# zz9tf/multimodal-fusion

Measured on AMD Instinct MI355X. Metric: similarity-pairs/sec (NxN cosine+top-k), higher is better.
Workload: dtype f16 MFMA scan + f32 exact re-rank; 1 GPU; N=262144 d=512 single-modality cosine + top-5, self excluded, f32 features, unit-norm Gaussian rows; rows_per_rank=262144, parallelism=single GPU, driver=single, scan_kernel=scan_b16x<f16> (v_mfma_f32_16x16x32_f16), col_splits=1, scan_grid=3088, fallback_rows=0, overflow_rows=0, query_order=False, near_duplicate_rows_estimate=0

## Files before the change

multimodal-fusion_amd/csrc/mmf_api.hip:

```cpp
#include <stdarg.h>
#include <string.h>

#include <algorithm>
#include <map>
#include <mutex>
#include <optional>
#include <utility>
#include <vector>

#include "mmf_host.h"

namespace mmf {

static thread_local char g_err[512] = "";

void set_error(const char* fmt, ...) {
  va_list ap;
  va_start(ap, fmt);
  vsnprintf(g_err, sizeof(g_err), fmt, ap);
  va_end(ap);
}

struct WsEntry { char* base = nullptr; size_t cap = 0; WsKept kept; };
static std::mutex g_ws_mu;
// ... 624 lines not shown
      else MMF_TRY(launch_scan_b16(sp, splits, L, scan_scratch, pn, s, &grid));
    } else {
      int list_base = 0;
      for (int p = 0; p < fo.n_panels; ++p) {
        const mmf_panel& P = fo.panels[p];
        if (P.ready_event) MMF_HIP(hipStreamWaitEvent(s, static_cast<hipEvent_t>(P.ready_event), 0));
        MMF_TRY(t_panel[p].start(profile, s));
        pn.list_base = list_base;
        list_base += 2 * panel_splits[p];
        pn.seg_len = (uint32_t)P.seg_len; pn.seg_stride = (uint32_t)P.seg_stride; pn.id_off = (uint32_t)P.id_base;
        sp.ZC = P.Z; sp.cb = P.cb; sp.m = P.m; sp.m_pad = P.m_pad;
        MMF_TRY(launch_scan_b16(sp, panel_splits[p], L, scan_scratch, pn, s, &grid));
        MMF_TRY(t_panel[p].stop(s));
      }
    }
    MMF_TRY(launch_scan_b16_audit(pn, L.overflow, n, s));
    if (const char* e = getenv("MMF_DEBUG_FLAG_ROWS")) {
      const int64_t f = atoll(e);
      if (f > 0) MMF_HIP(hipMemsetAsync(L.overflow, 1, (size_t)(f < n ? f : n) * 4, s));
    }
    MMF_TRY(t_scan.stop(s));
    if (symmetric && getenv("MMF_SYMMETRIC_DEBUG")) {
      MMF_HIP(hipStreamSynchronize(s));
      std::vector<uint32_t> hc((size_t)n), hl((size_t)sym_grid() * 8), hr((size_t)sym_grid() * 8);
      uint32_t none = 0;
      MMF_HIP(hipMemcpy(hc.data(), sym_cnt, hc.size() * 4, hipMemcpyDeviceToHost));
      MMF_HIP(hipMemcpy(hl.data(), sym.val_cnt, hl.size() * 4, hipMemcpyDeviceToHost));
      MMF_HIP(hipMemcpy(hr.data(), sym.log_cnt, hr.size() * 4, hipMemcpyDeviceToHost));
      MMF_HIP(hipMemcpy(&none, sym.none_cnt, 4, hipMemcpyDeviceToHost));
      unsigned long long tot = 0, logged = 0, records = 0; uint32_t mx = 0, lmx = 0;
      for (uint32_t v : hc) { tot += v; if (v > mx) mx = v; }
      for (uint32_t v : hl) logged += v;
      for (uint32_t v : hr) { records += v; if (v > lmx) lmx = v; }
      bool live, forward;
      symmetric_live_mode(&live, &forward);
      int phases; bool antipodal;
      symmetric_schedule_mode(&phases, &antipodal, sym_G);
      const size_t first_b = (size_t)sym_schedule_phase_b_begin((n + 255) / 256, sym_G) * 8;
      unsigned long long logged_b = 0;
      for (size_t i = first_b; i < hl.size(); ++i) logged_b += hl[i];
      fprintf(stderr, "[mmf symmetric] G %d grid %lld %s %s: rows without a threshold %u, received entries %llu (%.1f per row, largest %u of %d), fullest wave log %u of %d, logged entries %llu (%.1f per row, filing %s), records %llu, phases %d antipodal %d, logged by phase B %llu (%.1f per row)\n",
              sym_G, (long long)sym_grid(), live ? "live" : "frozen", forward ? "ahead" : "back", none, tot, (double)tot / (double)n, mx,
              kSymCap, lmx, scan_b16_sym_log_cap(), logged, (double)logged / (double)n, symmetric_prune_mode() ? "pruned" : "complete", records,
              forward ? 1 : phases, (antipodal && !forward) ? 1 : 0, logged_b, (double)logged_b / (double)n);
    }
    if (select_wait_event) MMF_HIP(hipStreamWaitEvent(s, static_cast<hipEvent_t>(select_wait_event), 0));

    SelectProblem q = r.select();
    q.rx = fo.rx; q.cy = fo.cy; q.perm = fo.perm;
    q.fail_rows = flags.fail_rows; q.fail_count = flags.fail_count; q.cand_total = r.stats ? flags.cand_total : nullptr;
    q.two_pass = true;
    q.order_scratch = getenv("MMF_SELECT_UNORDERED") ? nullptr : order_scratch;
    q.out_stride = out_stride;
    if (leave_floors) { q.floor_key_out = floor_key_out; q.floor_id_out = floor_id_out; }
    MMF_TRY(t_sel.start(profile, s));
    MMF_TRY(launch_select(q, L, s));
    MMF_TRY(t_sel.stop(s));

    MMF_TRY(flags.read(r.stats != nullptr, s));
    const uint32_t* h_fail4 = flags.h_fail4;
    const uint32_t h_fail = h_fail4[0];
    failed_rows = h_fail;
    if (h_fail > 0 && getenv("MMF_DEBUG_PRINT_FLAGGED")) {
      const uint32_t nshow = h_fail < 8 ? h_fail : 8;
      int32_t rows[8];
      MMF_HIP(hipMemcpy(rows, flags.fail_rows, nshow * sizeof(int32_t), hipMemcpyDeviceToHost));
      for (uint32_t i = 0; i < nshow; ++i) {
// ... 3898 lines not shown
```

multimodal-fusion_amd/csrc/mmf_host.h:

```cpp
#pragma once
#include <hip/hip_runtime.h>
#include <functional>
#include <optional>
#include <stdint.h>
#include <stdio.h>

#include <string>
#include <vector>

#include "../../include/mmf_hg.h"
#include "../../include/mmf_hg_topk.h"
#include "../../include/mmf_hg_topk16.h"
#include "../../include/ext/mmf_hg_topk16_seg.h"
#include "../../include/ext/mmf_hg_topk_xy.h"
#include "../../include/ext/mmf_hg_seg_exact.h"
#include "../../include/ext/mmf_hg_topk_anyk.h"
#include "../../include/ext/mmf_hg_kmeans_ragged.h"
#include "../../include/ext/mmf_hg_cross_seg.h"
#include "../../include/ext/mmf_hg_cross_seg16.h"
#include "../../include/ext/mmf_hg_cross_segw.h"
#include "../../include/ext/mmf_hg_fast_anyk.h"
#include "../../include/ext/mmf_hg_wide_anyk.h"
#include "../../include/ext/mmf_hg_seg_anyk.h"
#include "../../include/ext/mmf_hg_cross_seg_anyk.h"
// ... 129 lines not shown
  int spill_cap = 0;
  int spill_stacks = 0;
  uint32_t* sym_cnt = nullptr;
  uint2* sym_ent = nullptr;
  int sym_cap = 0;
};

constexpr int kSymListPairs = 3;
int64_t sym_schedule_grid(int64_t nb, int G);
int64_t sym_schedule_phase_b_begin(int64_t nb, int G);
void sym_schedule_table(int64_t nb, int G, int launch, int32_t* out, bool forward = false, int phases = 1, bool antipodal = false);
int sym_default_group(int64_t nb);
constexpr int kSymCap = 512;
constexpr int kSymLogPerWave = 2304;
int scan_b16_sym_log_cap();
struct SymBuffers {
  float* thr = nullptr;
  uint32_t* log = nullptr;
  uint32_t* log_cnt = nullptr;
  uint32_t* val_cnt = nullptr;
  int32_t* sched = nullptr;
  uint32_t* none_cnt = nullptr;
  static size_t bytes(int64_t n_pad, int64_t grid) {
    return ws_bytes(n_pad, 4) + ws_bytes((size_t)grid * 8 * kSymLogPerWave * 16, 4) + 2 * ws_bytes((size_t)grid * 8, 4) +
           ws_bytes((size_t)grid * 16, 4) + ws_bytes(4, 4);
  }
  void carve(Workspace& ws, int64_t n_pad, int64_t grid) {
    thr = ws.take<float>(n_pad); log = ws.take<uint32_t>((size_t)grid * 8 * kSymLogPerWave * 16);
    log_cnt = ws.take<uint32_t>((size_t)grid * 8); val_cnt = ws.take<uint32_t>((size_t)grid * 8); sched = ws.take<int32_t>((size_t)grid * 16); none_cnt = ws.take<uint32_t>(4);
  }
};

struct ScanB16Panel {
  int list_base = 0;
  uint32_t seg_len = 0, seg_stride = 0, id_off = 0;
  int32_t* seed = nullptr;
  int64_t seed_stride = 0;
  int share = 0;
  int32_t* sunk = nullptr;
};

int64_t prep_f32_rows(int64_t n);
int64_t prep_f32_dim(int64_t d);
size_t prep_f32_bytes(int64_t n, int64_t d);
int launch_prep_f32(const void* X, int64_t n, int64_t d, int dtype, const int32_t* row_ids, float* out, hipStream_t s);

struct ScanProblem {
  const void* X; int64_t n;
  const void* Y; int64_t m;
  const float* Xp = nullptr;
  const float* Yp = nullptr;
  int64_t d;
// ... 307 lines not shown
```

multimodal-fusion_amd/csrc/mmf_scan_bf16.hip:

```cpp
#include <stdlib.h>

#include <type_traits>

#include "mmf_dev.h"
#include "mmf_host.h"

namespace mmf {

constexpr int B_CT = 32;
#ifndef MMF_B_CAP
#define MMF_B_CAP 15
#endif
constexpr int B_CAP = MMF_B_CAP;
constexpr int B_CAP_BIG = 16;
constexpr int B_CAP_WIDE = 32;

typedef __bf16 bf16x8_t __attribute__((ext_vector_type(8)));
typedef _Float16 f16x8_t __attribute__((ext_vector_type(8)));
typedef uint32_t u32x4 __attribute__((ext_vector_type(4)));

struct PrepArgs {
  const void* X; int64_t n; int64_t d; int dtype; int metric;
  const float* scal;
  const uint32_t* max_n;
// ... 173 lines not shown
  const float g_chain = (float)(d + 2) * 5.9604645e-8f;
  const float slot_eps = (cap <= 16) ? 1.9073486e-6f : 3.8146973e-6f;
  const float e1 = rn * ZB + un * RB + (g_acc + slot_eps) * (zn * ZB + CB);
  float e2;
  if (metric == MMF_DOT) e2 = g_chain * un * UB;
  else if (metric == MMF_COSINE) e2 = (g_chain + 4.7683716e-7f) * un * UB * 1.01f;
  else e2 = g_chain * un * UB + 2.3841858e-7f * (un * un + UB * UB);
  return 2.0f * (e1 + e2) * 1.001f + 1e-30f;
}

__device__ __forceinline__ void glds4(const void* gptr, const void* lptr) {
  __builtin_amdgcn_global_load_lds((const __attribute__((address_space(1))) void*)(gptr), (__attribute__((address_space(3))) void*)(lptr), 4, 0, 0);
}

#ifndef MMF_SYM_ABLATE
#define MMF_SYM_ABLATE 0
#endif
#ifndef MMF_SYM_EARLY_THR
#define MMF_SYM_EARLY_THR 1
#endif
#ifndef MMF_SYM_RECORDS
#define MMF_SYM_RECORDS 1
#endif
#ifndef MMF_SYM_SCALAR_ANY
#define MMF_SYM_SCALAR_ANY 1
#endif
#ifndef MMF_SYM_ABLATE_Q
#define MMF_SYM_ABLATE_Q 0
#endif
#ifndef MMF_SYM_COUNT
#define MMF_SYM_COUNT 0
#endif
template <int KS, bool F16, bool DBG, int NW, int TPB, int CAP, bool SPLITK = false, bool SEG = false, int SYM = 0, bool XSEG = false,
          bool CEIL = false>
__global__ __launch_bounds__(64 * NW, (NW == 8) ? 2 : 1) void scan_b16x_kernel(ScanB16Args a) {
  static_assert(!CEIL || (SYM == 0 && !DBG), "per-row ceilings: the plain and the table-driven schedules (SEG, XSEG) only");
  static_assert(!SPLITK || (TPB == 1 && NW == 8 && (KS % 8) == 0), "split-k pairs");
  static_assert(SYM == 0 || (!SPLITK && !SEG && !DBG && TPB == 2), "symmetric schedule: the d = 512 kernel only");
  static_assert(!XSEG || (SEG && SYM == 0 && !DBG), "the cross-segment mask rides on the table-driven schedule");
  constexpr int NQW = SPLITK ? NW / 2 : NW;
  constexpr int NTL = 64 * NQW;
  constexpr int QT = 32 * NQW;
  constexpr int STAGES = 2 * TPB;
  constexpr int ROWB = KS * 32;
  constexpr int TILEB = B_CT * ROWB;
  constexpr int PIECES = TILEB / 1024;
// ... 70 lines not shown
    const float UB = __uint_as_float(a.maxima[2]), CB = __uint_as_float(a.maxima[3]);
    const float zn = a.q_zn[qop], rn = a.q_rn[qop], un = a.q_un[qop];
    const float g_acc = (float)(KS * 16 + 8) * 5.9604645e-8f;
    const float g_chain = (float)(a.d + 2) * 5.9604645e-8f;
    const float slot_eps = (CAP <= 16) ? 1.9073486e-6f : 3.8146973e-6f;
    const float e1 = rn * ZB + un * RB + (g_acc + slot_eps) * (zn * ZB + CB);
    float e2;
    if (a.metric == MMF_DOT) e2 = g_chain * un * UB;
    else if (a.metric == MMF_COSINE) e2 = (g_chain + 4.7683716e-7f) * un * UB * 1.01f;
    else e2 = g_chain * un * UB + 2.3841858e-7f * (un * un + UB * UB);
    margin = 2.0f * (e1 + e2) * 1.001f + 1e-30f;
  }

  SlotList<CAP, NTL> list;
  list.init(lkeys + (tid & (NTL - 1)), lids + (tid & (NTL - 1)));
  if (!qvalid) list.thr = __builtin_huge_valf();
  else if (a.spill_cnt) {
    list.sink.cnt = a.spill_cnt; list.sink.ids = a.spill_ids; list.sink.cap = (uint32_t)a.spill_cap; list.sink.row = qpos;
    list.sink.seg_len = a.seg_len; list.sink.seg_stride = a.seg_stride; list.sink.id_off = id_off;
    if (DBG) list.sink.ablate = (a.debug & 128) ? 1 : 0;
    if (a.spill_stacks) list.sink.stacks = 1 + half;
  }
  float pub = -kFltMax;
  auto sync_seed = [&]() {
    if (!qvalid) return;
    bool rose = false;
    if (list.thr > pub && list.thr > list.lost) {
      pub = list.thr;
      atomicMax(a.seed + qpos, seed_enc(pub));
      rose = true;
    }
    if (!a.share) return;
    const int32_t o = __hip_atomic_load(a.seed + qpos, __ATOMIC_RELAXED, __HIP_MEMORY_SCOPE_AGENT);
    if (o > kSeedNone) {
      const float t = __int_as_float(o >= 0 ? o : (o ^ 0x7fffffff));
      if (t > list.thr) { list.thr = t; pub = t; }
    }
    if constexpr (SYM == 2) {
      if (rose && a.sym_live) __hip_atomic_store(a.sym_thr + qpos, list.thr, __ATOMIC_RELAXED, __HIP_MEMORY_SCOPE_AGENT);
    }
  };
  constexpr bool SCALAR_ANY = SYM != 0 && MMF_SYM_SCALAR_ANY != 0;
  auto sym_hits = [&](unsigned long long b) -> bool { asm("" : "+s"(b)); return b != 0ull; };
  if (a.share) sync_seed();
  const bool seeded = !__any(list.thr == -kFltMax);

  constexpr int KS2 = SPLITK ? KS / 4 : KS / 2;
  const int kbyte = khalf * KS2 * 64;
  u32x4 qf[KS2][2];
  {
    const char* qbase = reinterpret_cast<const char*>(a.ZQ) + (q0 + 32 * qw + c16) * (int64_t)ROWB + g * 16 + kbyte;
#pragma unroll
    for (int s = 0; s < KS2; ++s) {
      qf[s][0] = *reinterpret_cast<const u32x4*>(qbase + s * 64);
      qf[s][1] = *reinterpret_cast<const u32x4*>(qbase + 16 * (int64_t)ROWB + s * 64);
    }
#pragma unroll
    for (int s = 0; s < KS2; ++s) { asm volatile("" : "+v"(qf[s][0])); asm volatile("" : "+v"(qf[s][1])); }
  }

  int lo[4];
#pragma unroll
  for (int j = 0; j < 4; ++j) lo[j] = c16 * ROWB + ((((4 * j + g) ^ c16) & 15) << 4);
// ... 6 lines not shown
    const int r = off / ROWB;
    const int chunk = (off % ROWB) >> 4;
    const int src_chunk = (chunk & ~15) | ((chunk ^ r) & 15);
    src_off[i] = (uint32_t)(r * ROWB + src_chunk * 16);
  }
  const char* zc0 = reinterpret_cast<const char*>(a.ZC) + (SYM != 0 ? 0 : t_begin * (int64_t)TILEB);
  const char* cb0 = reinterpret_cast<const char*>(a.cb + (SYM != 0 ? 0 : t_begin * B_CT));
  const char* zt0 = SYM != 0 ? zc0 + t_begin * (int64_t)TILEB : zc0;
  const char* ct0 = SYM != 0 ? cb0 + t_begin * B_CT * 4 : cb0;
  const __amdgpu_buffer_rsrc_t zrsrc = __builtin_amdgcn_make_buffer_rsrc(const_cast<char*>(zc0), 0, -1, 0x00020000);
  auto issue_piece = [&](const char* tsrc, int stage, int i) {
    if (DBG && (a.debug & 2)) return;
    if (DBG && (a.debug & 32)) tsrc = zc0;
    __builtin_amdgcn_raw_ptr_buffer_load_lds(zrsrc, (__attribute__((address_space(3))) void*)(tiles + stage * TILEB + (wave + NW * i) * 1024),
                                             16, (int)src_off[i], (int)(uint32_t)(tsrc - zc0), 0, 0);
  };
  const __amdgpu_buffer_rsrc_t brsrc = __builtin_amdgcn_make_buffer_rsrc(const_cast<char*>(cb0), 0, -1, 0x00020000);
  auto issue_bias = [&](const char* bsrc, int stage) {
    const uint32_t l = __builtin_amdgcn_mbcnt_hi(~0u, __builtin_amdgcn_mbcnt_lo(~0u, 0u));
    if (l < 32)
      __builtin_amdgcn_raw_ptr_buffer_load_lds(brsrc, (__attribute__((address_space(3))) void*)(cbs + stage * 64), 4, (int)(l * 4u),
                                               (int)(uint32_t)(bsrc - cb0), 0, 0);
  };
  auto sym_thr_stage = [&](int stage) -> float* { return lkeys + CAP * NTL + stage * 32; };
  auto issue_thr = [&](const char* bsrc, int stage) {
    const __amdgpu_buffer_rsrc_t trsrc = __builtin_amdgcn_make_buffer_rsrc(a.sym_thr, 0, -1, 0x00020000);
    const uint32_t l = __builtin_amdgcn_mbcnt_hi(~0u, __builtin_amdgcn_mbcnt_lo(~0u, 0u));
    if (l < 32)
      __builtin_amdgcn_raw_ptr_buffer_load_lds(trsrc, (__attribute__((address_space(3))) void*)sym_thr_stage(stage), 4, (int)(l * 4u),
                                               (int)(uint32_t)(bsrc - cb0), 0, 16);
  };

  auto issue_thr_pair = [&](const char* bsrc, int stage) {
    const __amdgpu_buffer_rsrc_t trsrc = __builtin_amdgcn_make_buffer_rsrc(a.sym_thr, 0, -1, 0x00020000);
    const uint32_t l = __builtin_amdgcn_mbcnt_hi(~0u, __builtin_amdgcn_mbcnt_lo(~0u, 0u));
    __builtin_amdgcn_raw_ptr_buffer_load_lds(trsrc, (__attribute__((address_space(3))) void*)sym_thr_stage(stage), 4, (int)(l * 4u),
                                             (int)(uint32_t)(bsrc - cb0), 0, 16);
  };

  if (SPLITK && tid < NQW) ack[tid] = -1;
  const int Ti = (int)T;
  if (Ti > 0) {
#pragma unroll
    for (int u = 0; u < TPB; ++u) {
      const bool real = u < Ti;
#pragma unroll
      for (int i = 0; i < PPW; ++i) issue_piece(real ? zt0 + u * (int64_t)TILEB : zc0, u, i);
      if constexpr (SYM == 0) { if (wave == (u & (NW - 1))) issue_bias(real ? ct0 + u * B_CT * 4 : cb0, u); }
      if constexpr (SYM == 2 && !MMF_SYM_EARLY_THR) { if (wave == ((u + 4) & (NW - 1))) issue_thr(real ? ct0 + u * B_CT * 4 : cb0, u); }
    }
    if constexpr (SYM == 2 && MMF_SYM_EARLY_THR) { if (wave == 4) issue_thr_pair(Ti >= TPB ? ct0 : cb0, 0); }
  }
  constexpr int GRP = KS2 / PPW;
  static_assert(KS2 % PPW == 0 && GRP >= 1, "DMA piece placement");
  const char* tsrc = zt0 + TPB * (int64_t)TILEB;
  const char* bsrc = ct0 + TPB * B_CT * 4;
  const uint32_t id_base = (uint32_t)(t_begin * B_CT);

// ... 127 lines not shown
        for (int r = 0; r < 16; ++r) nh += (v[r] >= list.thr) ? 1 : 0;
        const int lanes_hit = __popcll(__ballot(nh > 0));
#pragma unroll
        for (int o = 32; o > 0; o >>= 1) nh += __shfl_xor(nh, o);
        if (lane == 0) {
          atomicAdd(a.dbg + 0, 1ull);
          atomicAdd(a.dbg + 1, cold ? 1ull : 0ull);
          atomicAdd(a.dbg + 2, (unsigned long long)nh);
          atomicAdd(a.dbg + 3, (!cold && willc) ? 1ull : 0ull);
          atomicAdd(a.dbg + 4, (unsigned long long)lanes_hit);
        }
      }
      unsigned long long ts0 = 0;
      if (DBG && (a.debug & 16)) ts0 = __builtin_amdgcn_s_memtime();
      list.template offer_tile<!(DBG && SPLITK)>(v, id0, rowof, a.kk, margin);
      if (DBG && (a.debug & 16) && lane == 0) {
        const unsigned long long dt = __builtin_amdgcn_s_memtime() - ts0;
        atomicAdd(a.dbg + (cold ? 4 : 5), dt);
        atomicAdd(a.dbg + (cold ? 6 : 7), 1ull);
      }
      refresh_thr();
    }
    if (((DBG && (a.debug & 8)) || SYMCNT) && lane == 0) atomicAdd(a.dbg + 5, 1ull);
    if (__builtin_expect(a.share && (tt & 63) == 63, 0)) { sync_seed(); refresh_thr(); }
  };

  uint32_t sym_wcnt = 0;
  auto sym_offer = [&](const Acc& x, int tt, const float* th) {
    const f32x4 th0 = *reinterpret_cast<const f32x4*>(th + 4 * g);
    const f32x4 th1 = *reinterpret_cast<const f32x4*>(th + 16 + 4 * g);
    if constexpr (MMF_SYM_RECORDS != 0) {
      bool any0 = false, any1 = false;
      unsigned long long hit0 = 0ull, hit1 = 0ull;
#pragma unroll
      for (int j = 0; j < 4; ++j) {
        const bool p0 = fmaxf(x.t[0][0][j], x.t[0][1][j]) >= th0[j], p1 = fmaxf(x.t[1][0][j], x.t[1][1][j]) >= th1[j];
        any0 |= p0; any1 |= p1;
        if constexpr (SCALAR_ANY) { hit0 |= __builtin_amdgcn_ballot_w64(p0); hit1 |= __builtin_amdgcn_ballot_w64(p1); }
      }
      if (__builtin_expect((SCALAR_ANY ? sym_hits(hit0 | hit1) : __any(any0 || any1) != 0) && (MMF_SYM_ABLATE != 1 || a.sym_log_cap < 0), 0)) {
        const uint32_t cj0 = id_base + (uint32_t)tt * B_CT + ((tt >= sym_n1) ? (uint32_t)(sym_skip * B_CT) : 0u) + 4u * (uint32_t)g;
        const uint32_t qi0 = (uint32_t)(q0 + 32 * qw + c16);
        u32x4* lg = reinterpret_cast<u32x4*>(a.sym_log) + ((size_t)blockIdx.x * NW + wave) * (size_t)a.sym_log_cap * 4;
#pragma unroll
        for (int cb = 0; cb < 2; ++cb) {
          const bool hit = cb ? any1 : any0;
          const unsigned long long b = SCALAR_ANY ? (cb ? hit1 : hit0) : __ballot(hit);
          if (hit) {
            const uint32_t at = sym_wcnt + __builtin_amdgcn_mbcnt_hi((uint32_t)(b >> 32), __builtin_amdgcn_mbcnt_lo((uint32_t)b, 0u));
            if (at < (uint32_t)a.sym_log_cap) {
              if (MMF_SYM_ABLATE != 3) {
                u32x4 hd;
                hd[0] = cj0 + 16u * cb; hd[1] = qi0; hd[2] = 0u; hd[3] = 0u;
                u32x4* r = lg + (size_t)at * 4;
                r[0] = hd;
                r[1] = __builtin_bit_cast(u32x4, cb ? th1 : th0);
                r[2] = __builtin_bit_cast(u32x4, x.t[cb][0]);
                r[3] = __builtin_bit_cast(u32x4, x.t[cb][1]);
              }
            } else {
#pragma unroll
              for (int jj = 0; jj < 4; ++jj) {
                const uint32_t cj = cj0 + 16u * cb + jj;
                if ((int64_t)cj < a.n_rows) atomicMax(a.lost + cj, 0x7fffffff);
              }
            }
          }
          sym_wcnt += (uint32_t)__popcll(b);
        }
      }
      return;
    }
    bool any = false;
#pragma unroll
    for (int j = 0; j < 4; ++j) {
      any |= fmaxf(x.t[0][0][j], x.t[0][1][j]) >= th0[j];
      any |= fmaxf(x.t[1][0][j], x.t[1][1][j]) >= th1[j];
    }
    if (__builtin_expect(__any(any) && (MMF_SYM_ABLATE != 1 || a.sym_log_cap < 0), 0)) {
      const uint32_t cj0 = id_base + (uint32_t)tt * B_CT + ((tt >= sym_n1) ? (uint32_t)(sym_skip * B_CT) : 0u) + 4u * (uint32_t)g;
      const uint32_t qi0 = (uint32_t)(q0 + 32 * qw + c16);
      const bool sym_qv0 = q0 + 32 * qw + c16 < a.n_rows, sym_qv1 = q0 + 32 * qw + c16 + 16 < a.n_rows;
      uint32_t* lg = a.sym_log + ((size_t)blockIdx.x * NW + wave) * (size_t)a.sym_log_cap * 4;
      uint32_t m = 0;
#pragma unroll
      for (int cb = 0; cb < 2; ++cb) {
#pragma unroll
        for (int j = 0; j < 4; ++j) {
          const float tj = cb ? th1[j] : th0[j];
          const bool cv = (int64_t)(cj0 + 16u * cb + j) < a.n_rows;
          m |= (x.t[cb][0][j] >= tj && sym_qv0 && cv) ? (1u << (8 * cb + 2 * j)) : 0u;
          m |= (x.t[cb][1][j] >= tj && sym_qv1 && cv) ? (2u << (8 * cb + 2 * j)) : 0u;
        }
      }
      unsigned long long busy = __ballot(m != 0u);
      while (busy) {
        if (m != 0u) {
          const uint32_t b = (uint32_t)__builtin_ctz(m);
          m &= m - 1u;
          const float v = select16(b, x.t[0][0][0], x.t[0][1][0], x.t[0][0][1], x.t[0][1][1], x.t[0][0][2], x.t[0][1][2], x.t[0][0][3], x.t[0][1][3],
                                   x.t[1][0][0], x.t[1][1][0], x.t[1][0][1], x.t[1][1][1], x.t[1][0][2], x.t[1][1][2], x.t[1][0][3], x.t[1][1][3]);
          const uint32_t cj = cj0 + 16u * (b >> 3) + ((b >> 1) & 3u);
          const uint32_t at = sym_wcnt + __builtin_amdgcn_mbcnt_hi((uint32_t)(busy >> 32), __builtin_amdgcn_mbcnt_lo((uint32_t)busy, 0u));
          if (at < (uint32_t)a.sym_log_cap) {
            u32x4 ent;
            ent[0] = cj; ent[1] = qi0 + 16u * (b & 1u); ent[2] = __float_as_uint(v); ent[3] = 0u;
            if (MMF_SYM_ABLATE != 3) *reinterpret_cast<u32x4*>(lg + (size_t)at * 4) = ent;
          } else {
            atomicMax(a.lost + cj, 0x7fffffff);
          }
        }
        sym_wcnt += (uint32_t)__popcll(busy);
        busy = __ballot(m != 0u);
      }
    }
  };

  unsigned long long tw = 0, tf = 0, tc = 0, tv = 0, t0s = 0, t1s = 0, t2s = 0, t3s = 0, tvs = 0;
  const bool stamps = DBG && (a.debug & 16) != 0;
  Acc acc_prev;
  float m0_prev = kNegInf, m1_prev = kNegInf;
#pragma unroll
  for (int cb = 0; cb < 2; ++cb) {
#pragma unroll
    for (int j = 0; j < 4; ++j) { acc_prev.t[cb][0][j] = kNegInf; acc_prev.t[cb][1][j] = kNegInf; }
  }
  const int nIter = (Ti + TPB - 1) / TPB;
  for (int j = 0; j < nIter; ++j) {
    if (stamps) tvs = __builtin_amdgcn_s_memtime();
    __builtin_amdgcn_s_waitcnt(0x0F70);
    if (stamps) t0s = __builtin_amdgcn_s_memtime();
    asm volatile("" ::: "memory");
    if (!(DBG && (a.debug & 4)))
    __builtin_amdgcn_s_barrier();
    asm volatile("" ::: "memory");
    if (stamps) t1s = __builtin_amdgcn_s_memtime();

    if constexpr (SPLITK) {
      if (owner) {
        if (j > 0) {
#pragma unroll
          for (int i = 0; i < 4; ++i) {
            const f32x4 p = xch[(qw * 4 + i) * 64 + lane];
            acc_prev.t[i >> 1][i & 1] += p;
          }
          m0_prev = max_qb(acc_prev, 0);
          m1_prev = max_qb(acc_prev, 1);
        }
        asm volatile("" ::: "memory");
        if (lane == 0) ack[qw] = j;
      }
    }
    if (owner) filter(acc_prev, j * TPB - 1, m0_prev, m1_prev);
    if (stamps) t2s = __builtin_amdgcn_s_memtime();

    const int sg = (j & 1) * TPB, ng = TPB - sg;
#pragma unroll
    for (int u = 0; u < TPB; ++u) {
      const int t = j * TPB + u;
      const bool more = (t + TPB < Ti);
      const char* src = more ? tsrc + u * (int64_t)TILEB : zc0;
      Acc acc;
      acc = tile_body(tiles + (sg + u) * TILEB + kbyte, cbs + (sg + u) * 64, src, ng + u);
      if constexpr (SYM == 0) { if (wave == ((t + TPB) & (NW - 1))) issue_bias(more ? bsrc + u * B_CT * 4 : cb0, ng + u); }
      else mask_padding(acc, t);
      if constexpr (XSEG) mask_excluded(acc, t);
      if constexpr (SYM == 2 && MMF_SYM_ABLATE != 2) {
        if constexpr (MMF_SYM_EARLY_THR) { if (u == 0 && wave == (j & (NW - 1))) issue_thr_pair(more ? bsrc : cb0, ng); }
        else if (wave == ((t + TPB + 4) & (NW - 1))) issue_thr(more ? bsrc + u * B_CT * 4 : cb0, ng + u);
        if (t < Ti) sym_offer(acc, t, sym_thr_stage(sg + u));
      }
      if (u < TPB - 1) {
        if (TPB == 2 || __builtin_expect(t < Ti, 1))
        filter(acc, t, max_qb(acc, 0), max_qb(acc, 1));
      } else {
        if (__builtin_expect(t >= Ti, 0)) {
#pragma unroll
          for (int cb = 0; cb < 2; ++cb) {
#pragma unroll
            for (int jj = 0; jj < 4; ++jj) { acc.t[cb][0][jj] = kNegInf; acc.t[cb][1][jj] = kNegInf; }
          }
        }
        acc_prev = acc;
        if constexpr (!SPLITK) {
          m0_prev = max_qb(acc, 0);
          m1_prev = max_qb(acc, 1);
        } else if (!owner) {
          while (ack[qw] < j) __builtin_amdgcn_s_sleep(1);
          asm volatile("" ::: "memory");
#pragma unroll
          for (int i = 0; i < 4; ++i) xch[(qw * 4 + i) * 64 + lane] = acc.t[i >> 1][i & 1];
          __builtin_amdgcn_s_waitcnt(0xC07F);
        }
      }
    }
    tsrc += TPB * (int64_t)TILEB;
    bsrc += TPB * B_CT * 4;
    if constexpr (SYM != 0) {
      if ((j + 2) * TPB == sym_n1) { tsrc += sym_skip * (int64_t)TILEB; bsrc += sym_skip * (B_CT * 4); }
    }
    if (stamps) {
      asm volatile("" :: "v"(acc_prev.t[0][0][0]));
      t3s = __builtin_amdgcn_s_memtime();
      tw += t1s - t0s; tf += t2s - t1s; tc += t3s - t2s; tv += t0s - tvs;
    }
  }
  if (stamps && lane == 0) {
// ... 1 lines not shown
    atomicAdd(a.dbg + 8, tv);
  }
  if constexpr (SPLITK) {
    __builtin_amdgcn_s_waitcnt(0x0F70);
    __builtin_amdgcn_s_barrier();
    if (owner && Ti > 0) {
#pragma unroll
      for (int i = 0; i < 4; ++i) acc_prev.t[i >> 1][i & 1] += xch[(qw * 4 + i) * 64 + lane];
    }
  }
  if (Ti > 0 && owner) filter(acc_prev, nIter * TPB - 1, max_qb(acc_prev, 0), max_qb(acc_prev, 1));
  __builtin_amdgcn_s_waitcnt(0x0F70);

  list.compact(a.kk, margin);
  list.sink.close();
  if (a.spill_stacks && a.spill_cnt) {
    const uint32_t mine = qvalid ? list.sink.cpos : 0u;
    const uint32_t theirs = (uint32_t)__shfl_xor((int)mine, 32);
    if (mine + theirs > (uint32_t)a.spill_cap) list.lost = kFltMax;
    if (qvalid && half == 0 && (mine | theirs)) a.spill_cnt[qpos] = mine | (theirs << 16);
  }
  sync_seed();
  if constexpr (SYM == 2) {
    if (MMF_SYM_ABLATE == 3) sym_wcnt = 0;
    if (lane == 0) a.sym_log_cnt[(size_t)blockIdx.x * NW + wave] = sym_wcnt < (uint32_t)a.sym_log_cap ? sym_wcnt : (uint32_t)a.sym_log_cap;
  }
  if (qvalid) {
    const int64_t lbase = qpos * a.lists_total + a.list_base + 2 * split + half;
    a.cand_cnt[lbase] = (uint32_t)list.cnt;
    for (int e = 0; e < list.cnt; ++e) {
      uint32_t id = list.id_of(e);
      if (a.seg_len) id = (id / a.seg_len) * a.seg_stride + id % a.seg_len;
      a.cand_ids[lbase * CAP + e] = id + id_off;
      if (a.cand_keys) a.cand_keys[lbase * CAP + e] = list.keys[e * NTL];
    }
    if (a.cand_keys && half == 0) a.margin_out[qpos] = margin;
    if (list.lost > kNegInf) atomicMax(a.lost + qpos, seed_enc(list.lost) + SlotList<CAP, NTL>::SLOTS);
  }
  if (SYM != 0 && (MMF_SYM_ABLATE_Q & SYM) != 0 && (MMF_SYM_ABLATE_Q & 4) != 0) lids[tid & (NTL - 1)] = __float_as_uint(ablate_keep);
}

__global__ void audit_kernel(const int32_t* seed, const int32_t* lost, uint32_t* overflow, int64_t n) {
  const int64_t i = (int64_t)blockIdx.x * blockDim.x + threadIdx.x;
  if (i >= n) return;
  const int32_t l = lost[i];
  if (l > kSeedNone && l >= seed[i]) overflow[i] = 1u;
}

// ... 45 lines not shown
}

int scan_bf16_cap(int kk, int dp) {
  if (dp > 512) return B_CAP;
  return kk <= B_CAP - 4 ? B_CAP : (kk <= 20 ? B_CAP_BIG : B_CAP_WIDE);
}
int scan_bf16_slot_ulp(int cap) { return cap <= 16 ? 16 : 32; }
int scan_bf16_dp(int64_t d) { return pad_dp(d); }

int launch_prep_half(const PrepRows& r, const HalfImage& out, int dp, bool f16, hipStream_t s) {
  return launch_prep_half_gather(r, nullptr, r.n, out, dp, f16, s);
}

int launch_prep_half_gather(const PrepRows& r, const int32_t* gather, int64_t n_pos, const HalfImage& out, int dp, bool f16, hipStream_t s) {
  PrepArgs a{r.X, n_pos, r.d, r.dtype, r.metric, r.scal, r.max_n, out.Z, out.n_pad, dp, f16 ? 1 : 0, out.zn, out.rn, out.un, out.cb,
             out.maxima, gather};
  int64_t grid = (out.n_pad + 3) / 4;
  if (grid > 1024) grid = 1024;
  hipLaunchKernelGGL(prep_half_kernel, dim3((unsigned)grid), dim3(256), 0, s, a);
  MMF_LAUNCH_CHECK();
  return MMF_OK;
}

static size_t scan_b16_lds(int ks, int nw, int tpb, int cap, bool splitk, bool sym_thr = false) {
  const int nqw = splitk ? nw / 2 : nw;
  return (size_t)(2 * tpb) * (B_CT * ks * 32) + (size_t)(2 * tpb) * 64 * 4 + (size_t)cap * (64 * nqw) * 4 +
         (splitk ? (size_t)nqw * 4 * 64 * 16 + 64 : 0) + (sym_thr ? (size_t)(2 * tpb) * 32 * 4 : 0);
}

int scan_b16_queries_per_block(int dp) { return 32 * waves_for_dp(dp); }

static int conc_splits_for(int64_t row_blocks, int col_splits) {
  int cs = 1;
  while (cs < 8 && cs < col_splits && row_blocks * cs < 256) cs <<= 1;
  return cs;
}
static int64_t scan_b16_round_blocks(int64_t row_blocks, int cs) {
  const int per = 8 / cs;
  return ((row_blocks + per - 1) / per) * 8;
}
static int64_t scan_b16_grid(int64_t n_rows, int col_splits, int dp) {
  const int qt = scan_b16_queries_per_block(dp);
  const int64_t row_blocks = (n_rows + qt - 1) / qt;
  const int cs = conc_splits_for(row_blocks, col_splits);
  return scan_b16_round_blocks(row_blocks, cs) * (col_splits / cs);
}

size_t scan_b16_scratch_bytes(int64_t n_rows, int col_splits, int dp, int cap) {
  return (size_t)scan_b16_grid(n_rows, col_splits, dp) * (cap <= 16 ? 16 : 32) * (64 * waves_for_dp(dp)) * 4 + 256;
}

template <int KS, int NW, int TPB, int CAP, bool SPLITK = false, bool SEG = false, int SYM = 0, bool XSEG = false, bool CEIL = false>
static int launch_b16_t(const ScanB16Args& a, bool f16, int64_t grid, hipStream_t s) {
  const size_t lds = scan_b16_lds(KS, NW, TPB, CAP, SPLITK, SYM == 2);
  auto go = [&](auto kern) -> int {
    MMF_HIP(hipFuncSetAttribute(reinterpret_cast<const void*>(kern), hipFuncAttributeMaxDynamicSharedMemorySize, (int)lds));
    hipLaunchKernelGGL(kern, dim3((unsigned)grid), dim3(64 * NW), lds, s, a);
    MMF_LAUNCH_CHECK();
    return MMF_OK;
  };
  if constexpr (SEG || SYM != 0 || CEIL) {
    if (f16) return go(scan_b16x_kernel<KS, true, false, NW, TPB, CAP, SPLITK, SEG, SYM, XSEG, CEIL>);
    return go(scan_b16x_kernel<KS, false, false, NW, TPB, CAP, SPLITK, SEG, SYM, XSEG, CEIL>);
  }
  if (a.debug != 0) {
    if (f16) return go(scan_b16x_kernel<KS, true, true, NW, TPB, CAP, SPLITK>);
    return go(scan_b16x_kernel<KS, false, true, NW, TPB, CAP, SPLITK>);
  }
  if (f16) return go(scan_b16x_kernel<KS, true, false, NW, TPB, CAP, SPLITK>);
  return go(scan_b16x_kernel<KS, false, false, NW, TPB, CAP, SPLITK>);
}

template <bool SEG, bool XSEG = false, bool CEIL = false>
static int launch_b16_for(const char* who, int dp, int cap, const ScanB16Args& a, bool f16, int64_t grid, hipStream_t s) {
  const bool big = (cap == B_CAP_BIG);
  if (cap == B_CAP_WIDE) {
    switch (dp) {
// ... 243 lines not shown
        int64_t lo = forward ? sb + 1 : sb - h, hi = lo + h - 1;
        if (phases == 2) { if (lo < 0) lo = 0; }
        else {
          if (lo >= ns) { lo -= ns; hi -= ns; }
          if (lo < 0) { lo += ns; hi += ns; }
        }
        if (hi < lo) continue;
        if (hi < ns) { b1 = first_tile(lo); n1 = end_tile(hi) - b1; }
        else { b1 = first_tile(lo); n1 = end_tile(ns - 1) - b1; b2 = 0; n2 = end_tile(hi - ns); }
      }
      if (anti) {
        const int64_t o = sb - ns / 2;
        if (n1 == 0) { b1 = first_tile(o); n1 = end_tile(o) - b1; }
        else { b2 = first_tile(o); n2 = end_tile(o) - b2; }
      }
    }
    if (n2 == 0) b2 = b1 + n1;
    e[SYM_RB] = (int32_t)rbi; e[SYM_B1] = (int32_t)b1; e[SYM_N1] = (int32_t)n1; e[SYM_B2] = (int32_t)b2; e[SYM_N2] = (int32_t)n2;
    e[SYM_SLOT] = phase_b ? 1 : 0;
    e[SYM_PHASE] = launch == 0 || phases != 2 ? 0 : (phase_b ? 2 : 1);
  }
}

__global__ void sym_thr_kernel(const int32_t* seed, float* thr, int64_t n, int64_t n_pad, uint32_t* none_cnt) {
  const int64_t i = (int64_t)blockIdx.x * blockDim.x + threadIdx.x;
  if (i >= n_pad) return;
  if (i >= n) { thr[i] = __builtin_huge_valf(); return; }
  const int32_t o = seed[i];
  if (o > kSeedNone) { thr[i] = __int_as_float(o >= 0 ? o : (o ^ 0x7fffffff)); return; }
  thr[i] = -kFltMax;
  atomicAdd(none_cnt, 1u);
}

__global__ __launch_bounds__(256) void sym_scatter_kernel(const uint32_t* log, const uint32_t* log_cnt, int log_cap, uint32_t* sym_cnt,
                                                          uint2* sym_ent, int cap, int32_t* lost,
                                                          const int32_t* seed, int slot_ulp, int64_t n_rows, uint32_t* val_cnt) {
  const uint32_t c = log_cnt[blockIdx.x];
#if MMF_SYM_RECORDS
  __shared__ uint32_t passed_all;
  if (c == 0) { if (threadIdx.x == 0) val_cnt[blockIdx.x] = 0u; return; }
  if (threadIdx.x == 0) passed_all = 0u;
  __syncthreads();
  const uint32_t* lg = log + (size_t)blockIdx.x * log_cap * 16;
  uint32_t passed = 0;
  for (uint32_t e = threadIdx.x; e < 8u * c; e += 256) {
    const uint32_t* r = lg + (size_t)(e >> 3) * 16;
    const uint32_t vi = e & 7u, j = vi & 3u;
    const uint32_t cj = r[0] + j, qi = r[1] + 16u * (vi >> 2), kb = r[8 + vi];
    if (!(__uint_as_float(kb) >= __uint_as_float(r[4 + j])) || (int64_t)qi >= n_rows || (int64_t)cj >= n_rows) continue;
    ++passed;
    if (seed) {
      const int32_t sd = seed[cj], b = (int32_t)kb;
      if (sd > kSeedNone && (b >= 0 ? b : (b ^ 0x7fffffff)) + slot_ulp < sd) continue;
    }
// ... 38 lines not shown
size_t scan_b16_sym_scratch_bytes(int64_t n_rows, int G) {
  const int64_t nb = (n_rows + 255) / 256;
  return (size_t)sym_schedule_grid(nb, G) * 16 * 512 * 4 + 256;
}

int launch_scan_b16_sym(const ScanB16Problem& p, const SymLaunch& y, const CandLists& L, void* scratch, const SymBuffers& sb,
                        const ScanB16Panel& pn, hipStream_t s, int* grid_out) {
  const int64_t n = p.n_rows, nb = (n + 255) / 256, n_pad = nb * 256, grid = sym_schedule_grid(nb, y.G);
  const int log_cap = scan_b16_sym_log_cap();
  if (p.metric != MMF_DOT && p.metric != MMF_COSINE) {
    set_error("scan_b16_sym: metric %d has a per-candidate bias, which the symmetric kernels do not apply", p.metric);
    return MMF_E_INTERNAL;
  }
  if (L.lists != 2 * kSymListPairs || L.cap != B_CAP || !L.keys || !L.margin || !L.sym_cnt || !pn.seed) { set_error("scan_b16_sym: lists missing"); return MMF_E_INTERNAL; }
  if (n_pad * 1024 >= (int64_t(1) << 32)) { set_error("scan_b16_sym: operand image beyond the 32-bit tile offsets"); return MMF_E_INTERNAL; }
  if (y.tables) {
    std::vector<int32_t> tab((size_t)grid * 2 * SEG_ENTRY);
    sym_schedule_table(nb, y.G, 0, tab.data(), y.forward, y.phases, y.antipodal);
    sym_schedule_table(nb, y.G, 1, tab.data() + (size_t)grid * SEG_ENTRY, y.forward, y.phases, y.antipodal);
    MMF_TRY(upload_table(s, sb.sched, tab.data(), tab.size() * 4));
  }
  MMF_HIP(hipMemsetAsync(L.sym_cnt, 0, (size_t)n * 4, s));
  MMF_HIP(hipMemsetAsync(L.cnt, 0, (size_t)n * L.lists * 4, s));
  MMF_HIP(hipMemsetAsync(sb.log_cnt, 0, (size_t)grid * 8 * 4, s));
  MMF_HIP(hipMemsetAsync(sb.none_cnt, 0, 16, s));
  ScanB16Args a = scan_args(p, L, pn, scratch);
  a.ZQ = p.ZC;
  a.tiles_total = n_pad / B_CT; a.row_blocks = nb;
  a.spill_stacks = 0;
  a.sched = sb.sched;
  a.sym_thr = sb.thr; a.sym_live = y.live ? 1 : 0; a.sym_log = sb.log; a.sym_log_cnt = sb.log_cnt; a.sym_log_cap = log_cap;
#if MMF_SYM_COUNT
  static unsigned long long* dbuf = nullptr;
  if (!dbuf) MMF_HIP(hipMalloc(&dbuf, 128));
  a.dbg = dbuf;
  auto report = [&](int launch) -> int {
    unsigned long long h[8];
    MMF_HIP(hipMemcpyAsync(h, dbuf, 64, hipMemcpyDeviceToHost, s));
    MMF_HIP(hipStreamSynchronize(s));
    fprintf(stderr, "[mmf sym count] launch %d: wave-tiles=%llu visits=%llu (cold %llu) hits=%llu entry-compactions=%llu lanes-with-hit=%llu\n",
            launch, h[5], h[0], h[1], h[2], h[3], h[4]);
    return MMF_OK;
  };
  MMF_HIP(hipMemsetAsync(dbuf, 0, 128, s));
#endif
  MMF_TRY((launch_b16_t<32, 8, 2, B_CAP, false, false, 1>(a, p.f16, grid, s)));
#if MMF_SYM_COUNT
  MMF_TRY(report(0));
  MMF_HIP(hipMemsetAsync(dbuf, 0, 128, s));
#endif
  hipLaunchKernelGGL(sym_thr_kernel, dim3((unsigned)((n_pad + 255) / 256)), dim3(256), 0, s, pn.seed, sb.thr, n, n_pad, sb.none_cnt);
  MMF_LAUNCH_CHECK();
  a.sched = sb.sched + (size_t)grid * SEG_ENTRY; a.list_base = 2; a.share = 1;
  MMF_TRY((launch_b16_t<32, 8, 2, B_CAP, false, false, 2>(a, p.f16, grid, s)));
#if MMF_SYM_COUNT
  MMF_TRY(report(1));
#endif
  hipLaunchKernelGGL(sym_scatter_kernel, dim3((unsigned)(grid * 8)), dim3(256), 0, s, sb.log, sb.log_cnt, log_cap, L.sym_cnt,
                     L.sym_ent, L.sym_cap, pn.seed + pn.seed_stride, y.prune ? pn.seed : nullptr, L.slot_ulp, n, sb.val_cnt);
  MMF_LAUNCH_CHECK();
  if (grid_out) *grid_out = (int)(2 * grid);
  return MMF_OK;
}

// ... 2 lines not shown
```

Baseline: 2198 billion pairs/s.

## Add coarse group-minimum prefilter to symmetric scan threshold offers

The threshold kernel now also writes, for each 32-column tile, the minimum threshold of each group of four rows. The second symmetric scan pass loads these minima together with the per-row thresholds in the same paired DMA, and skips the detailed per-element threshold compare and logging whenever a wave's tile maximum cannot beat any group minimum. To fit the extra loads, the threshold staging moves into the bias stages' LDS. The pass also publishes refreshed group minima when seeds rise, and the per-iteration waitcnt is loosened under a chain-wait flag. This trades a few shuffles, atomic stores and LDS reads per tile for skipping most record work, at the cost of extra memory-ordering subtlety.

```diff
diff --git a/multimodal-fusion_amd/csrc/mmf_api.hip b/multimodal-fusion_amd/csrc/mmf_api.hip
--- a/multimodal-fusion_amd/csrc/mmf_api.hip
+++ b/multimodal-fusion_amd/csrc/mmf_api.hip
@@ -670,16 +670,17 @@
     MMF_TRY(t_scan.stop(s));
     if (symmetric && getenv("MMF_SYMMETRIC_DEBUG")) {
       MMF_HIP(hipStreamSynchronize(s));
-      std::vector<uint32_t> hc((size_t)n), hl((size_t)sym_grid() * 8), hr((size_t)sym_grid() * 8);
+      std::vector<uint32_t> hc((size_t)n), hl((size_t)sym_grid() * 8), hr((size_t)sym_grid() * 24);
       uint32_t none = 0;
       MMF_HIP(hipMemcpy(hc.data(), sym_cnt, hc.size() * 4, hipMemcpyDeviceToHost));
       MMF_HIP(hipMemcpy(hl.data(), sym.val_cnt, hl.size() * 4, hipMemcpyDeviceToHost));
       MMF_HIP(hipMemcpy(hr.data(), sym.log_cnt, hr.size() * 4, hipMemcpyDeviceToHost));
       MMF_HIP(hipMemcpy(&none, sym.none_cnt, 4, hipMemcpyDeviceToHost));
-      unsigned long long tot = 0, logged = 0, records = 0; uint32_t mx = 0, lmx = 0;
+      unsigned long long tot = 0, logged = 0, records = 0, coarse = 0, hit_tiles = 0; uint32_t mx = 0, lmx = 0;
       for (uint32_t v : hc) { tot += v; if (v > mx) mx = v; }
       for (uint32_t v : hl) logged += v;
-      for (uint32_t v : hr) { records += v; if (v > lmx) lmx = v; }
+      const size_t waves = hl.size();
+      for (size_t i = 0; i < waves; ++i) { records += hr[i]; if (hr[i] > lmx) lmx = hr[i]; coarse += hr[waves + i]; hit_tiles += hr[2 * waves + i]; }
       bool live, forward;
       symmetric_live_mode(&live, &forward);
       int phases; bool antipodal;
@@ -687,10 +688,10 @@
       const size_t first_b = (size_t)sym_schedule_phase_b_begin((n + 255) / 256, sym_G) * 8;
       unsigned long long logged_b = 0;
       for (size_t i = first_b; i < hl.size(); ++i) logged_b += hl[i];
-      fprintf(stderr, "[mmf symmetric] G %d grid %lld %s %s: rows without a threshold %u, received entries %llu (%.1f per row, largest %u of %d), fullest wave log %u of %d, logged entries %llu (%.1f per row, filing %s), records %llu, phases %d antipodal %d, logged by phase B %llu (%.1f per row)\n",
+      fprintf(stderr, "[mmf symmetric] G %d grid %lld %s %s: rows without a threshold %u, received entries %llu (%.1f per row, largest %u of %d), fullest wave log %u of %d, logged entries %llu (%.1f per row, filing %s), records %llu, phases %d antipodal %d, logged by phase B %llu (%.1f per row), coarse visits %llu, hit wave-tiles %llu\n",
               sym_G, (long long)sym_grid(), live ? "live" : "frozen", forward ? "ahead" : "back", none, tot, (double)tot / (double)n, mx,
               kSymCap, lmx, scan_b16_sym_log_cap(), logged, (double)logged / (double)n, symmetric_prune_mode() ? "pruned" : "complete", records,
-              forward ? 1 : phases, (antipodal && !forward) ? 1 : 0, logged_b, (double)logged_b / (double)n);
+              forward ? 1 : phases, (antipodal && !forward) ? 1 : 0, logged_b, (double)logged_b / (double)n, coarse, hit_tiles);
     }
     if (select_wait_event) MMF_HIP(hipStreamWaitEvent(s, static_cast<hipEvent_t>(select_wait_event), 0));
 
diff --git a/multimodal-fusion_amd/csrc/mmf_host.h b/multimodal-fusion_amd/csrc/mmf_host.h
--- a/multimodal-fusion_amd/csrc/mmf_host.h
+++ b/multimodal-fusion_amd/csrc/mmf_host.h
@@ -175,12 +175,12 @@
   int32_t* sched = nullptr;
   uint32_t* none_cnt = nullptr;
   static size_t bytes(int64_t n_pad, int64_t grid) {
-    return ws_bytes(n_pad, 4) + ws_bytes((size_t)grid * 8 * kSymLogPerWave * 16, 4) + 2 * ws_bytes((size_t)grid * 8, 4) +
-           ws_bytes((size_t)grid * 16, 4) + ws_bytes(4, 4);
+    return ws_bytes(n_pad + n_pad / 8, 4) + ws_bytes((size_t)grid * 8 * kSymLogPerWave * 16, 4) + ws_bytes((size_t)grid * 24, 4) +
+           ws_bytes((size_t)grid * 8, 4) + ws_bytes((size_t)grid * 16, 4) + ws_bytes(4, 4);
   }
   void carve(Workspace& ws, int64_t n_pad, int64_t grid) {
-    thr = ws.take<float>(n_pad); log = ws.take<uint32_t>((size_t)grid * 8 * kSymLogPerWave * 16);
-    log_cnt = ws.take<uint32_t>((size_t)grid * 8); val_cnt = ws.take<uint32_t>((size_t)grid * 8); sched = ws.take<int32_t>((size_t)grid * 16); none_cnt = ws.take<uint32_t>(4);
+    thr = ws.take<float>(n_pad + n_pad / 8); log = ws.take<uint32_t>((size_t)grid * 8 * kSymLogPerWave * 16);
+    log_cnt = ws.take<uint32_t>((size_t)grid * 24); val_cnt = ws.take<uint32_t>((size_t)grid * 8); sched = ws.take<int32_t>((size_t)grid * 16); none_cnt = ws.take<uint32_t>(4);
   }
 };
 
diff --git a/multimodal-fusion_amd/csrc/mmf_scan_bf16.hip b/multimodal-fusion_amd/csrc/mmf_scan_bf16.hip
--- a/multimodal-fusion_amd/csrc/mmf_scan_bf16.hip
+++ b/multimodal-fusion_amd/csrc/mmf_scan_bf16.hip
@@ -219,6 +219,15 @@
 #ifndef MMF_SYM_RECORDS
 #define MMF_SYM_RECORDS 1
 #endif
+#ifndef MMF_SYM_COARSE
+#define MMF_SYM_COARSE 1
+#endif
+#if MMF_SYM_COARSE && !MMF_SYM_EARLY_THR
+#error "MMF_SYM_COARSE: the group minima ride on the paired threshold DMA (MMF_SYM_EARLY_THR=1)"
+#endif
+#ifndef MMF_SYM_CHAIN_WAIT
+#define MMF_SYM_CHAIN_WAIT 1
+#endif
 #ifndef MMF_SYM_SCALAR_ANY
 #define MMF_SYM_SCALAR_ANY 1
 #endif
@@ -335,6 +344,7 @@
     if (a.spill_stacks) list.sink.stacks = 1 + half;
   }
   float pub = -kFltMax;
+  bool seed_rose = false;
   auto sync_seed = [&]() {
     if (!qvalid) return;
     bool rose = false;
@@ -350,8 +360,23 @@
       if (t > list.thr) { list.thr = t; pub = t; }
     }
     if constexpr (SYM == 2) {
-      if (rose && a.sym_live) __hip_atomic_store(a.sym_thr + qpos, list.thr, __ATOMIC_RELAXED, __HIP_MEMORY_SCOPE_AGENT);
-    }
+      if (rose && a.sym_live) {
+        uint32_t off = (uint32_t)qpos * 4u;
+        asm volatile("" : "+v"(off));
+        __hip_atomic_store(reinterpret_cast<float*>(reinterpret_cast<char*>(a.sym_thr) + off), list.thr, __ATOMIC_RELAXED, __HIP_MEMORY_SCOPE_AGENT);
+        seed_rose = true;
+      }
+    }
+  };
+  auto sync_tmin = [&]() {
+    if (__any(seed_rose)) {
+      float v = qvalid ? pub : __builtin_huge_valf();
+      v = fminf(v, __shfl_xor(v, 1)); v = fminf(v, __shfl_xor(v, 2));
+      v = fminf(v, __shfl_xor(v, 16)); v = fminf(v, __shfl_xor(v, 32));
+      if ((lane & 0x33) == 0)
+        __hip_atomic_store(a.sym_thr + a.tiles_total * B_CT + ((q0 >> 5) + qw) * 4 + (c16 >> 2), v, __ATOMIC_RELAXED, __HIP_MEMORY_SCOPE_AGENT);
+    }
+    seed_rose = false;
   };
   constexpr bool SCALAR_ANY = SYM != 0 && MMF_SYM_SCALAR_ANY != 0;
   auto sym_hits = [&](unsigned long long b) -> bool { asm("" : "+s"(b)); return b != 0ull; };
@@ -404,7 +429,10 @@
       __builtin_amdgcn_raw_ptr_buffer_load_lds(brsrc, (__attribute__((address_space(3))) void*)(cbs + stage * 64), 4, (int)(l * 4u),
                                                (int)(uint32_t)(bsrc - cb0), 0, 0);
   };
-  auto sym_thr_stage = [&](int stage) -> float* { return lkeys + CAP * NTL + stage * 32; };
+  constexpr int SYM_GRP = 2 * B_CT + 8;
+  static_assert(SYM != 2 || (2 * SYM_GRP <= STAGES * 64 && TPB == 2), "thresholds and group minima in the bias stages");
+  auto sym_thr_stage = [&](int stage) -> float* { return cbs + (stage >> 1) * SYM_GRP + (stage & 1) * B_CT; };
+  auto sym_min_stage = [&](int stage) -> float* { return cbs + (stage >> 1) * SYM_GRP + 2 * B_CT + (stage & 1) * 4; };
   auto issue_thr = [&](const char* bsrc, int stage) {
     const __amdgpu_buffer_rsrc_t trsrc = __builtin_amdgcn_make_buffer_rsrc(a.sym_thr, 0, -1, 0x00020000);
     const uint32_t l = __builtin_amdgcn_mbcnt_hi(~0u, __builtin_amdgcn_mbcnt_lo(~0u, 0u));
@@ -416,6 +444,12 @@
   auto issue_thr_pair = [&](const char* bsrc, int stage) {
     const __amdgpu_buffer_rsrc_t trsrc = __builtin_amdgcn_make_buffer_rsrc(a.sym_thr, 0, -1, 0x00020000);
     const uint32_t l = __builtin_amdgcn_mbcnt_hi(~0u, __builtin_amdgcn_mbcnt_lo(~0u, 0u));
+    if constexpr (MMF_SYM_COARSE != 0) {
+      const uint32_t off = (uint32_t)(bsrc - cb0);
+      const uint32_t voff = l < 16u ? off + l * 16u : (uint32_t)a.tiles_total * (B_CT * 4u) + (off >> 3) + (l - 16u) * 16u;
+      if (l < 18u)
+        __builtin_amdgcn_raw_ptr_buffer_load_lds(trsrc, (__attribute__((address_space(3))) void*)sym_thr_stage(stage), 16, (int)voff, 0, 0, 16);
+    } else
     __builtin_amdgcn_raw_ptr_buffer_load_lds(trsrc, (__attribute__((address_space(3))) void*)sym_thr_stage(stage), 4, (int)(l * 4u),
                                              (int)(uint32_t)(bsrc - cb0), 0, 16);
   };
@@ -589,11 +623,21 @@
       refresh_thr();
     }
     if (((DBG && (a.debug & 8)) || SYMCNT) && lane == 0) atomicAdd(a.dbg + 5, 1ull);
-    if (__builtin_expect(a.share && (tt & 63) == 63, 0)) { sync_seed(); refresh_thr(); }
+    if (__builtin_expect(a.share && (tt & 63) == 63, 0)) {
+      sync_seed();
+      if constexpr (SYM == 2 && MMF_SYM_COARSE != 0) sync_tmin();
+      refresh_thr();
+    }
   };
 
-  uint32_t sym_wcnt = 0;
-  auto sym_offer = [&](const Acc& x, int tt, const float* th) {
+  uint32_t sym_wcnt = 0, sym_cvis = 0, sym_htile = 0;
+  auto sym_offer = [&](const Acc& x, int tt, const float* th, float tmn, float mm) {
+    if constexpr (MMF_SYM_COARSE != 0) {
+      if (__builtin_expect(!(SCALAR_ANY ? sym_hits(__builtin_amdgcn_ballot_w64(mm >= tmn)) : __any(mm >= tmn) != 0) ||
+                           (MMF_SYM_ABLATE == 4 && a.sym_log_cap >= 0), 1)) return;
+      ++sym_cvis;
+      if (SYMCNT && lane == 0) atomicAdd(a.dbg + 6, 1ull);
+    }
     const f32x4 th0 = *reinterpret_cast<const f32x4*>(th + 4 * g);
     const f32x4 th1 = *reinterpret_cast<const f32x4*>(th + 16 + 4 * g);
     if constexpr (MMF_SYM_RECORDS != 0) {
@@ -609,6 +653,8 @@
         const uint32_t cj0 = id_base + (uint32_t)tt * B_CT + ((tt >= sym_n1) ? (uint32_t)(sym_skip * B_CT) : 0u) + 4u * (uint32_t)g;
         const uint32_t qi0 = (uint32_t)(q0 + 32 * qw + c16);
         u32x4* lg = reinterpret_cast<u32x4*>(a.sym_log) + ((size_t)blockIdx.x * NW + wave) * (size_t)a.sym_log_cap * 4;
+        ++sym_htile;
+        if (SYMCNT && lane == 0) atomicAdd(a.dbg + 7, 1ull);
 #pragma unroll
         for (int cb = 0; cb < 2; ++cb) {
           const bool hit = cb ? any1 : any0;
@@ -649,6 +695,7 @@
       const uint32_t qi0 = (uint32_t)(q0 + 32 * qw + c16);
       const bool sym_qv0 = q0 + 32 * qw + c16 < a.n_rows, sym_qv1 = q0 + 32 * qw + c16 + 16 < a.n_rows;
       uint32_t* lg = a.sym_log + ((size_t)blockIdx.x * NW + wave) * (size_t)a.sym_log_cap * 4;
+      ++sym_htile;
       uint32_t m = 0;
 #pragma unroll
       for (int cb = 0; cb < 2; ++cb) {
@@ -695,6 +742,9 @@
   const int nIter = (Ti + TPB - 1) / TPB;
   for (int j = 0; j < nIter; ++j) {
     if (stamps) tvs = __builtin_amdgcn_s_memtime();
+    if constexpr (SYM == 2 && MMF_SYM_CHAIN_WAIT != 0) {
+      __builtin_amdgcn_s_waitcnt(0x0070);
+    } else
     __builtin_amdgcn_s_waitcnt(0x0F70);
     if (stamps) t0s = __builtin_amdgcn_s_memtime();
     asm volatile("" ::: "memory");
@@ -728,6 +778,12 @@
       const bool more = (t + TPB < Ti);
       const char* src = more ? tsrc + u * (int64_t)TILEB : zc0;
       Acc acc;
+      constexpr bool COARSE = SYM == 2 && MMF_SYM_COARSE != 0 && MMF_SYM_ABLATE != 2;
+      float tmn = 0.f, m0 = 0.f, m1 = 0.f;
+      if constexpr (COARSE) {
+        tmn = sym_min_stage(sg + u)[g];
+        __builtin_amdgcn_sched_group_barrier(0x100, 1, 0);
+      }
       acc = tile_body(tiles + (sg + u) * TILEB + kbyte, cbs + (sg + u) * 64, src, ng + u);
       if constexpr (SYM == 0) { if (wave == ((t + TPB) & (NW - 1))) issue_bias(more ? bsrc + u * B_CT * 4 : cb0, ng + u); }
       else mask_padding(acc, t);
@@ -735,11 +791,12 @@
       if constexpr (SYM == 2 && MMF_SYM_ABLATE != 2) {
         if constexpr (MMF_SYM_EARLY_THR) { if (u == 0 && wave == (j & (NW - 1))) issue_thr_pair(more ? bsrc : cb0, ng); }
         else if (wave == ((t + TPB + 4) & (NW - 1))) issue_thr(more ? bsrc + u * B_CT * 4 : cb0, ng + u);
-        if (t < Ti) sym_offer(acc, t, sym_thr_stage(sg + u));
+        if constexpr (COARSE) { m0 = max_qb(acc, 0); m1 = max_qb(acc, 1); }
+        if (t < Ti) sym_offer(acc, t, sym_thr_stage(sg + u), tmn, fmaxf(m0, m1));
       }
       if (u < TPB - 1) {
         if (TPB == 2 || __builtin_expect(t < Ti, 1))
-        filter(acc, t, max_qb(acc, 0), max_qb(acc, 1));
+        filter(acc, t, COARSE ? m0 : max_qb(acc, 0), COARSE ? m1 : max_qb(acc, 1));
       } else {
         if (__builtin_expect(t >= Ti, 0)) {
 #pragma unroll
@@ -747,9 +804,12 @@
 #pragma unroll
             for (int jj = 0; jj < 4; ++jj) { acc.t[cb][0][jj] = kNegInf; acc.t[cb][1][jj] = kNegInf; }
           }
+          m0 = kNegInf; m1 = kNegInf;
         }
         acc_prev = acc;
-        if constexpr (!SPLITK) {
+        if constexpr (COARSE) {
+          m0_prev = m0; m1_prev = m1;
+        } else if constexpr (!SPLITK) {
           m0_prev = max_qb(acc, 0);
           m1_prev = max_qb(acc, 1);
         } else if (!owner) {
@@ -797,8 +857,13 @@
   }
   sync_seed();
   if constexpr (SYM == 2) {
+    if constexpr (MMF_SYM_COARSE != 0) sync_tmin();
     if (MMF_SYM_ABLATE == 3) sym_wcnt = 0;
-    if (lane == 0) a.sym_log_cnt[(size_t)blockIdx.x * NW + wave] = sym_wcnt < (uint32_t)a.sym_log_cap ? sym_wcnt : (uint32_t)a.sym_log_cap;
+    if (lane == 0) {
+      uint32_t* lc = a.sym_log_cnt + (size_t)blockIdx.x * NW + wave;
+      lc[0] = sym_wcnt < (uint32_t)a.sym_log_cap ? sym_wcnt : (uint32_t)a.sym_log_cap;
+      lc[(size_t)gridDim.x * NW] = sym_cvis; lc[2 * (size_t)gridDim.x * NW] = sym_htile;
+    }
   }
   if (qvalid) {
     const int64_t lbase = qpos * a.lists_total + a.list_base + 2 * split + half;
@@ -890,10 +955,10 @@
   return MMF_OK;
 }
 
-static size_t scan_b16_lds(int ks, int nw, int tpb, int cap, bool splitk, bool sym_thr = false) {
+static size_t scan_b16_lds(int ks, int nw, int tpb, int cap, bool splitk) {
   const int nqw = splitk ? nw / 2 : nw;
   return (size_t)(2 * tpb) * (B_CT * ks * 32) + (size_t)(2 * tpb) * 64 * 4 + (size_t)cap * (64 * nqw) * 4 +
-         (splitk ? (size_t)nqw * 4 * 64 * 16 + 64 : 0) + (sym_thr ? (size_t)(2 * tpb) * 32 * 4 : 0);
+         (splitk ? (size_t)nqw * 4 * 64 * 16 + 64 : 0);
 }
 
 int scan_b16_queries_per_block(int dp) { return 32 * waves_for_dp(dp); }
@@ -920,7 +985,7 @@
 
 template <int KS, int NW, int TPB, int CAP, bool SPLITK = false, bool SEG = false, int SYM = 0, bool XSEG = false, bool CEIL = false>
 static int launch_b16_t(const ScanB16Args& a, bool f16, int64_t grid, hipStream_t s) {
-  const size_t lds = scan_b16_lds(KS, NW, TPB, CAP, SPLITK, SYM == 2);
+  const size_t lds = scan_b16_lds(KS, NW, TPB, CAP, SPLITK);
   auto go = [&](auto kern) -> int {
     MMF_HIP(hipFuncSetAttribute(reinterpret_cast<const void*>(kern), hipFuncAttributeMaxDynamicSharedMemorySize, (int)lds));
     hipLaunchKernelGGL(kern, dim3((unsigned)grid), dim3(64 * NW), lds, s, a);
@@ -1210,14 +1275,26 @@
   }
 }
 
-__global__ void sym_thr_kernel(const int32_t* seed, float* thr, int64_t n, int64_t n_pad, uint32_t* none_cnt) {
-  const int64_t i = (int64_t)blockIdx.x * blockDim.x + threadIdx.x;
-  if (i >= n_pad) return;
-  if (i >= n) { thr[i] = __builtin_huge_valf(); return; }
-  const int32_t o = seed[i];
-  if (o > kSeedNone) { thr[i] = __int_as_float(o >= 0 ? o : (o ^ 0x7fffffff)); return; }
-  thr[i] = -kFltMax;
-  atomicAdd(none_cnt, 1u);
+__global__ __launch_bounds__(256) void sym_thr_kernel(const int32_t* seed, float* thr, int64_t n, int64_t n_pad, uint32_t* none_cnt) {
+  __shared__ float sv[256];
+  const int64_t i = (int64_t)blockIdx.x * 256 + threadIdx.x;
+  float v = __builtin_huge_valf();
+  if (i < n) {
+    const int32_t o = seed[i];
+    if (o > kSeedNone) v = __int_as_float(o >= 0 ? o : (o ^ 0x7fffffff));
+    else { v = -kFltMax; atomicAdd(none_cnt, 1u); }
+  }
+  if (i < n_pad) thr[i] = v;
+  sv[threadIdx.x] = v;
+  __syncthreads();
+  const int64_t t = (int64_t)blockIdx.x * 8 + (threadIdx.x >> 2);
+  if (threadIdx.x < 32 && t * B_CT < n_pad) {
+    const float* r = sv + (threadIdx.x >> 2) * B_CT + 4 * (threadIdx.x & 3);
+    float m = __builtin_huge_valf();
+#pragma unroll
+    for (int jj = 0; jj < 4; ++jj) m = fminf(m, fminf(r[jj], r[16 + jj]));
+    thr[n_pad + 4 * t + (threadIdx.x & 3)] = m;
+  }
 }
 
 __global__ __launch_bounds__(256) void sym_scatter_kernel(const uint32_t* log, const uint32_t* log_cnt, int log_cap, uint32_t* sym_cnt,
@@ -1302,7 +1379,7 @@
   }
   MMF_HIP(hipMemsetAsync(L.sym_cnt, 0, (size_t)n * 4, s));
   MMF_HIP(hipMemsetAsync(L.cnt, 0, (size_t)n * L.lists * 4, s));
-  MMF_HIP(hipMemsetAsync(sb.log_cnt, 0, (size_t)grid * 8 * 4, s));
+  MMF_HIP(hipMemsetAsync(sb.log_cnt, 0, (size_t)3 * grid * 8 * 4, s));
   MMF_HIP(hipMemsetAsync(sb.none_cnt, 0, 16, s));
   ScanB16Args a = scan_args(p, L, pn, scratch);
   a.ZQ = p.ZC;
@@ -1315,11 +1392,11 @@
   if (!dbuf) MMF_HIP(hipMalloc(&dbuf, 128));
   a.dbg = dbuf;
   auto report = [&](int launch) -> int {
-    unsigned long long h[8];
-    MMF_HIP(hipMemcpyAsync(h, dbuf, 64, hipMemcpyDeviceToHost, s));
+    unsigned long long h[16];
+    MMF_HIP(hipMemcpyAsync(h, dbuf, 128, hipMemcpyDeviceToHost, s));
     MMF_HIP(hipStreamSynchronize(s));
-    fprintf(stderr, "[mmf sym count] launch %d: wave-tiles=%llu visits=%llu (cold %llu) hits=%llu entry-compactions=%llu lanes-with-hit=%llu\n",
-            launch, h[5], h[0], h[1], h[2], h[3], h[4]);
+    fprintf(stderr, "[mmf sym count] launch %d: wave-tiles=%llu visits=%llu (cold %llu) hits=%llu entry-compactions=%llu lanes-with-hit=%llu coarse-visits=%llu hit-wave-tiles=%llu\n",
+            launch, h[5], h[0], h[1], h[2], h[3], h[4], h[6], h[7]);
     return MMF_OK;
   };
   MMF_HIP(hipMemsetAsync(dbuf, 0, 128, s));
```

Result: faster. 2229 billion pairs/s, median of 6 (+1.4%).
